# lenke182/flood-uav-video-segmentation

Measured on AMD Instinct MI355X. Metric: segmentation FPS @713x713 (PSPNet-ResNet50 keyframe + linear interp, frame_delta=5), higher is better.
Workload: dtype f32

## Files before the change

### flood_uav_video_segmentation_amd/csrc/kernels.h

```cpp
#pragma once
#include "common.h"

namespace fs {

struct ConvParams {
    const float* in;    int ld_in;
    const float* wgt;
    int ld_wgt;
    const float* scale;
    const float* shift;
    const float* res;   int ld_res;
    float* out;         int ld_out;
    int B, H, W, Cin;
    int Ho, Wo, Cout;
    int KH, KW, stride, pad, dil;
    const float* in2;   int ld_in2;
    int Cin2, stride2, H2, W2;
    int relu;
    int res_touch;
    int korder;
    int groups;
    long long g_in, g_wgt, g_out;
    const void* wgt3;
    unsigned plane_bytes;
    unsigned short* kv_k;
    unsigned short* kv_vt;
    int kv_N, kv_Npad, kv_heads;
    unsigned kv_plane_bytes;
    int kv_b;
};
int launch_conv_igemm(const ConvParams& p, hipStream_t s, int tile = 0);
const char* conv_igemm_tile_name(const ConvParams& p, int tile = 0);
int launch_split_bf16x3(const float* w, long long n, void* planes, hipStream_t s);

static inline int conv_out_size(int in, int k, int stride, int pad, int dil) { return (in + 2 * pad - dil * (k - 1) - 1) / stride + 1; }
static inline ConvParams conv2d_params(const float* in, int ld_in, const float* wgt, const float* scale, const float* shift, const float* res, int ld_res,
                                       float* out, int ld_out, int B, int H, int W, int Cin, int Cout, int KH, int KW, int stride, int pad, int dil,
                                       int relu, int korder) {
    ConvParams p{};
    p.in = in; p.ld_in = ld_in; p.wgt = wgt; p.scale = scale; p.shift = shift; p.res = res; p.ld_res = ld_res; p.out = out; p.ld_out = ld_out;
    p.B = B; p.H = H; p.W = W; p.Cin = Cin; p.Cout = Cout;
    p.Ho = conv_out_size(H, KH, stride, pad, dil);
    p.Wo = conv_out_size(W, KW, stride, pad, dil);
    p.KH = KH; p.KW = KW; p.stride = stride; p.pad = pad; p.dil = dil; p.relu = relu; p.korder = korder;
    return p;
}
static inline ConvParams gemm_params(const float* in, int ld_in, const float* w, float* out, int ld_out, int rows, int K, int N) {
    return conv2d_params(in, ld_in, w, nullptr, nullptr, nullptr, 0, out, ld_out, 1, rows, 1, K, N, 1, 1, 1, 0, 1, 0, 0);
}
static inline void attach_planes(ConvParams& p, const void* planes, size_t elems) {
    p.wgt3 = planes;
    p.plane_bytes = (unsigned)(elems * 2);
}

struct FrameSrc {
    const float* in;
    const float* in2;
    int B1;
    int ncrops, FH, FW;
    short cy[32], cx[32];
};
static inline FrameSrc frames_plain(const float* in, const float* in2, int B1) {
    FrameSrc f{};
    f.in = in;
    f.in2 = in2;
    f.B1 = B1;
    return f;
}

struct StemParams {
    FrameSrc src;
    const float* wgt;
    const float* scale; const float* shift;
    float* out; int ld_out;
    int B, H, W, Ho, Wo, Cout, KH, KW, stride, pad;
    int split;
};
int launch_stem_conv(const StemParams& p, hipStream_t s);
static inline StemParams stem_params(const FrameSrc& src, const float* wgt, const float* scale, const float* shift, float* out, int B, int H, int W,
                                     int Cout, int KH, int KW, int stride, int pad, int split) {
    StemParams p{};
    p.src = src; p.wgt = wgt; p.scale = scale; p.shift = shift; p.out = out; p.ld_out = Cout;
    p.B = B; p.H = H; p.W = W; p.Cout = Cout; p.KH = KH; p.KW = KW; p.stride = stride; p.pad = pad; p.split = split;
    p.Ho = conv_out_size(H, KH, stride, pad, 1);
    p.Wo = conv_out_size(W, KW, stride, pad, 1);
    return p;
}

int launch_maxpool3x3s2(const float* in, int ld_in, float* out, int ld_out, int B, int H, int W, int C,
                        int Ho, int Wo, hipStream_t s);

int launch_adaptive_avgpool(const float* in, int ld_in, float* out, int B, int H, int W, int C, int bin,
                            hipStream_t s);

int launch_ppm_pool_combine(const float* cell_mean, float* out1, float* out2, float* out3, int B, int C, hipStream_t s);

int launch_rowdot_1x1(const float* in, int ld_in, const float* wgt, const float* scale, const float* shift,
                      float* out, int ld_out, int M, int K, int N, int relu, hipStream_t s);
struct RowdotProblem { const float* in; const float* wgt; const float* scale; const float* shift; float* out; int M; };
struct RowdotBatch { RowdotProblem p[4]; };
int launch_rowdot_1x1_batch(const RowdotBatch& pb, int nprob, int ld_in, int ld_out, int K, int N, int relu, hipStream_t s);

int launch_upsample_into(const float* in, int hi, int wi, float* out, int ld_out, int B, int Ho, int Wo,
                         int C, int align_corners, hipStream_t s);

int launch_classifier_nchw(const float* in, int ld_in, const float* wgt , const float* bias,
                           float* out , int B, int HW, int C, int K, hipStream_t s);

int launch_pack_oihw_to_ohwi(const float* w, float* out, int O, int I, int KH, int KW, hipStream_t s);
int launch_pack_oihw_to_hwio(const float* w, float* out, int O, int I, int KH, int KW, hipStream_t s);
int launch_pack_oihw_chunk_major(const float* w, float* out, int O, int I, int KH, int KW, hipStream_t s);
int launch_pack_slice_tap_major(const float* w, float* out, int O, int I, int c0, int nc, int taps, hipStream_t s);
size_t ppm_term_scratch_floats(int B, int H, int C);
int launch_ppm_term_classify(const float* T, int ld, const float* const Z[4], const int bins[4], float* scratch, const float* scale,
                             const float* shift, int B, int H, int W, int C, int relu, const float* cls_w , const float* cls_b,
                             float* logits_nchw, int K, hipStream_t s);
int launch_concat_scaled_filters(const float* wa, const float* sa, const float* ha, int Ka, const float* wb, const float* sb, const float* hb,
                                 int Kb, float* out, float* shift_out, int O, hipStream_t s);
int launch_nchw_to_nhwc(const float* in, float* out, int ld_out, int B, int C, int HW, hipStream_t s);
int launch_nhwc_to_nchw(const float* in, int ld_in, float* out, int B, int C, int HW, hipStream_t s);

int launch_grid_sample_nchw(const float* in, int B, int C, int Hi, int Wi, const float* grid, int Hg, int Wg,
                            float* out, int align_corners, hipStream_t s);
int launch_grid_sample_nhwc(const float* in, int ld_in, int B, int C, int Hi, int Wi, const float* grid, int Hg,
                            int Wg, float* out, int ld_out, int align_corners, hipStream_t s);
int launch_resize_bilinear_nchw(const float* in, int BC, int Hi, int Wi, float* out, int Ho, int Wo,
                                int align_corners, hipStream_t s);
int launch_resize_bilinear_nhwc(const float* in, int ld_in, int B, int C, int Hi, int Wi, float* out, int ld_out,
                                int Ho, int Wo, int align_corners, hipStream_t s, int max_blocks = 16384);
int launch_blend(const float* a, float wa, const float* b, float wb, float* out, int64_t numel, hipStream_t s);

struct SegFuseArgs {
    const float* lo_prev;
    const float* lo_next;
    const float* const* grids_left;
    const float* const* grids_right;
    int K, h, w;
    int Hg, Wg;
    int H, W;
    int n;
    int no_warp;
    float* out_logits;
    uint8_t* out_mask;
    float* scratch;
    double* canvas;
    double* count;
    int cH, cW, y0, x0;
};
struct SegTailParams : SegFuseArgs {
    const float* weights;
};
int launch_seg_tail(const SegTailParams& p, hipStream_t s);

struct FeatTailParams {
    const float* f_prev;
    const float* f_next;
    const float* const* grids_left;
    const float* const* grids_right;
    const float* grid0;
    int C, fh, fw, Hg, Wg, H0, W0, n, no_warp;
    float* stack;
    float* scratch;
    const float* weights;
};
int launch_feat_tail(const FeatTailParams& p, hipStream_t s);

struct CropsFuseArgs {
    const float* lo_prev;
    const float* lo_next;
    const float* scratch;
    int nc;
    short cy[64], cx[64];
    int K, h, w, Hg, Wg, ch, cw, n, no_warp;
    double* canvas;
    uint8_t* mask;
    int H, W;
    float sy_lo, sx_lo, sy_g, sx_g;
};
struct CropsFuseParams : CropsFuseArgs {
    const float* weights;
};
int launch_crops_fuse(CropsFuseParams p, const float* grids, float* scratch, hipStream_t s);

int launch_ms_prepare(const float* raw, int H, int W, int new_h, int new_w, int PH, int PW, const float* mean, const float* std, float* out,
                      int flip, hipStream_t s);
struct MsFuseParams {
    const float* lo_plain;
    const float* lo_flip;
    int nc;
    short cy[64], cx[64];
    int K, h, w, ch, cw;
    int PH, PW, new_h, new_w;
    double* scaled;
    int pad_top, pad_left;
    float sy_lo, sx_lo;
};
int launch_ms_fuse(MsFuseParams p, double* pred, int H, int W, int scale_index, int nscales, uint8_t* mask, hipStream_t s);

int launch_argmax_u8(const float* in, int B, int K, int64_t HW, uint8_t* out, hipStream_t s);
int launch_resize_argmax_u8(const float* in, int B, int K, int Hi, int Wi, uint8_t* out, int Ho, int Wo,
                            hipStream_t s);
int launch_softmax_accumulate(const float* logits, int n, int K, int h, int w, double* canvas, double* count, int H, int W, int y0,
                              int x0, hipStream_t s);
int launch_canvas_finish(double* canvas, const double* count, int n, int K, int64_t HW, uint8_t* mask, hipStream_t s);
int launch_resize_crop(const float* in, int B, int K, int Hi, int Wi, int Hfull, int Wfull, int align_corners, float* logits,
                       uint8_t* mask, int Ho, int Wo, hipStream_t s);
int launch_canvas_resize_argmax(const double* canvas, int n, int K, int Hi, int Wi, uint8_t* mask, int Ho, int Wo, hipStream_t s);
struct CropGridParams {
    const float* grids[32];
    int ngrids, Hg, Wg;
    int H, W;
    int ncrops, fh, fw;
    int ng_total, g0;
    short bho[32], bwo[32], bh[32], bw[32];
    float off_h[32], off_w[32], den_h[32], den_w[32];
    float* out;
};
int launch_crop_grids(const CropGridParams& p, hipStream_t s);
int launch_colorize(const uint8_t* mask, const uint8_t* palette, int K, uint8_t* rgb, int64_t numel, hipStream_t s);
int launch_mv_to_grids(const int* mv, int n, int stride, int hb, int wb, int bs, int H, int W, int* owners, double* grid,
                       double* inv_grid, hipStream_t s);
int launch_block_match(const uint8_t* cur, const uint8_t* ref, int H, int W, int channels, int R, int lambda, int* mv, int* cost,
                       hipStream_t s);
int launch_block_match_modes(const uint8_t* cur, const uint8_t* ref, int H, int W, int channels, int R, int lambda, int intra_bias, int cut_permille,
                             int* mv, int* cost, int* activity, int* stats, hipStream_t s);
constexpr int WINDOW_MAX_FRAMES = 64;
int launch_window_weights(const int* const* stats, int n, float* weights, int* source, hipStream_t s);
int launch_frame_prepare(const uint8_t* frame, const uint8_t* u, const uint8_t* v, int format, int matrix, int full_range, int H, int W,
                         const float* mean, const float* std, float* out, int h, int w, hipStream_t s);
int launch_frame_compose(const uint8_t* mask, int h, int w, const uint8_t* palette, int K, const uint8_t* frame, const uint8_t* u, const uint8_t* v,
                         int format, int matrix, int full_range, int H, int W, uint8_t* out, uint8_t* out_u, uint8_t* out_v, int out_format,
                         int out_matrix, int out_full_range, hipStream_t s);
int launch_iou_hist(const uint8_t* pred, const uint8_t* target, int64_t numel, int K, int ignore_index,
                    long long* hist3K, hipStream_t s);
int launch_mask_confidence(const float* logits, int n, int K, int h, int w, uint8_t* mask, uint8_t* conf, int H, int W, hipStream_t s);
int launch_canvas_confidence(const double* canvas, int n, int K, int Hi, int Wi, uint8_t* mask, uint8_t* conf, int Ho, int Wo, hipStream_t s);
int launch_frame_report(const uint8_t* mask, const uint8_t* conf, int n, int H, int W, int K, int low, long long* out, hipStream_t s);

int region_rank_chunks(int H, int W);
int launch_mask_regions(const uint8_t* mask, int n, int H, int W, int K, int connectivity, int* labels, hipStream_t s);
int launch_region_table(const uint8_t* mask, const int* labels, const uint8_t* conf, int n, int H, int W, int K, int low, int max_regions,
                        long long* table, long long* counts, int* index, int* workspace, hipStream_t s);
int launch_region_filter(const uint8_t* mask, const int* index, const long long* table, int n, int H, int W, int K, int max_regions,
                         int min_area, uint8_t* out, int* votes, hipStream_t s);


int launch_patchify(const float* in, const float* in2, int B1, float* out, int B, int H, int W, int P, int gh, int gw, hipStream_t s);
int launch_vit_assemble(const float* emb, const float* cls, const float* pos, float* X, int B, int N, int D, hipStream_t s);
int launch_dec_assemble(const float* Y, const float* cls_emb, float* Z, int B, int N, int K, int D, hipStream_t s);
int launch_layernorm(const float* in, const float* gamma, const float* beta, float* out, int rows, int D, int rows_per_batch,
                     int drop_first, hipStream_t s);
size_t attention_scratch_floats(int B, int N, int heads);
int launch_attention_f32(const float* qkv, float* out, int B, int N, int heads, float scale, float* scratch, hipStream_t s);
size_t attention_split_floats(int B, int N, int heads);
int launch_attention_split(const float* qkv, float* out, int B, int N, int heads, float scale, float* scratch, float* planes, hipStream_t s, bool planes_ready = false);
int launch_splitk_combine(const float* part, int nsplit, const float* bias, const float* res, float* out, int rows, int N, hipStream_t s);
int launch_splitk_combine_ln(const float* part, int nsplit, const float* bias, const float* res, float* out, const float* gamma, const float* beta,
                             float* ln_out, int rows, int N, hipStream_t s);
int launch_mask_head(const float* pp, const float* cc, const float* gamma, const float* beta, float* out, int B, int N, int K,
                     int D, hipStream_t s);


int launch_winograd_filter(const float* w, float* U , int O, int I, int mt, hipStream_t s, int chunk_major = 0);
int launch_winograd_input(const float* in, int ld_in, float* V , int B, int H, int W, int C, int dil, int mt,
                          hipStream_t s);
int launch_winograd_output(const float* M , const float* scale, const float* shift, float* out, int ld_out, int B,
                           int H, int W, int N, int relu, int dil, int mt, hipStream_t s);
struct WinoLayout { bool tile_major; long long s_pos, s_tile; };
WinoLayout winograd_layout(int mt, long long T, int C);
static inline ConvParams winograd_gemm_params(const float* V, const float* U, float* M, int mt, int T, int Cin, int Cout) {
    ConvParams p = gemm_params(V, Cin, U, M, Cout, T, Cin, Cout);
    const WinoLayout a = winograd_layout(mt, T, Cin), o = winograd_layout(mt, T, Cout);
    p.ld_in = (int)a.s_tile;
    p.g_in = a.s_pos;
    p.ld_out = (int)o.s_tile;
    p.g_out = o.s_pos;
    p.groups = (mt + 2) * (mt + 2);
    p.g_wgt = (long long)Cout * Cin;
    return p;
}
static inline size_t wino_v_floats(int mt, size_t T, int Cin, size_t align) { return ((size_t)(mt + 2) * (mt + 2) * T * Cin + align - 1) / align * align; }
static inline size_t wino_vm_floats(int mt, size_t T, int Cin, int Cout, size_t align) {
    return wino_v_floats(mt, T, Cin, align) + (size_t)(mt + 2) * (mt + 2) * T * Cout;
}
static inline int winograd_tiles(int B, int H, int W, int dil, int mt) {
    return B * dil * dil * ((cdiv(H, dil) + mt - 1) / mt) * ((cdiv(W, dil) + mt - 1) / mt);
}
static inline double winograd_gemm_rows(int B, int H, int W, int dil, int mt) {
    return (double)(mt + 2) * (mt + 2) * (double)(cdiv(winograd_tiles(B, H, W, dil, mt), 64) * 64);
}
static inline int winograd_pick_m(int , int H, int W, int dil) {
    const int m = winograd_gemm_rows(1, H, W, dil, 6) < winograd_gemm_rows(1, H, W, dil, 4) ? 6 : 4;
    return winograd_gemm_rows(1, H, W, dil, 3) < winograd_gemm_rows(1, H, W, dil, m) ? 3 : m;
}
static inline int wino_m(int force, int H, int W, int dil) { return force ? force : winograd_pick_m(1, H, W, dil); }

size_t wino_fused_bank_floats(int Cin, int Cout);
bool wino_fused_supported(int Cin, int Cout, int KH, int KW, int stride, int pad, int dil);
int launch_wino4_filter_packed(const float* w, float* U, int O, int I, hipStream_t s, int chunk_major = 0);
int launch_wino4_fused(const float* in, int ld_in, const float* U, const float* scale, const float* shift, float* out, int ld_out, int B, int H,
                       int W, int Cin, int Cout, int relu, hipStream_t s, int variant = 0);

int launch_wino4_fused_pool(const float* in, int ld_in, const float* U, const float* scale, const float* shift, float* pool, int ld_pool, int B,
                            int H, int W, int Cin, int Cout, hipStream_t s);

}
```

### flood_uav_video_segmentation_amd/csrc/wino_fused.hip

```cpp
#include "kernels.h"
#include "winograd.h"

namespace fs {

__device__ __forceinline__ int wf_voff(int m, int k) {
    const int g = (0x78 >> ((m >> 1) & 6)) & 3;
    return m * 16 + 4 * ((k >> 2) ^ g) + (k & 3);
}

__device__ __forceinline__ void wf_bt(const float d[6], float t[6]) {
    const float s12 = d[1] + d[2], d12 = d[1] - d[2], s34 = d[3] + d[4], d43 = d[4] - d[3], d42 = d[4] - d[2], d31 = d[3] - d[1];
    t[0] = __builtin_fmaf(4.f, d[0], __builtin_fmaf(-5.f, d[2], d[4]));
    t[1] = __builtin_fmaf(-4.f, s12, s34);
    t[2] = __builtin_fmaf(4.f, d12, d43);
    t[3] = __builtin_fmaf(2.f, d31, d42);
    t[4] = __builtin_fmaf(-2.f, d31, d42);
    t[5] = __builtin_fmaf(4.f, d[1], __builtin_fmaf(-5.f, d[3], d[5]));
}
__device__ __forceinline__ void wf_at(const float m[6], float y[4]) {
    const float s12 = m[1] + m[2], d12 = m[1] - m[2], s34 = m[3] + m[4], d34 = m[3] - m[4];
    y[0] = (m[0] + s12) + s34;
    y[1] = __builtin_fmaf(2.f, d34, d12);
    y[2] = __builtin_fmaf(4.f, s34, s12);
    y[3] = __builtin_fmaf(8.f, d34, d12) + m[5];
}

__global__ __launch_bounds__(256) void wino4_filter_packed_kernel(const float* __restrict__ w, float* __restrict__ U, int O, int I, int chunk_major) {
    const int64_t total = (int64_t)O * I;
    const int ts = chunk_major ? 32 : 1;
    for (int64_t i = (int64_t)blockIdx.x * 256 + threadIdx.x; i < total; i += (int64_t)gridDim.x * 256) {
        const int o = (int)(i / I), c = (int)(i - (int64_t)o * I);
        const float* g = chunk_major ? w + (i >> 5) * 288 + (i & 31) : w + i * 9;
        double t[6][3];
#pragma unroll
        for (int s = 0; s < 3; ++s) {
            double col[6];
            Wino<4>::g(g[(0 * 3 + s) * ts], g[(1 * 3 + s) * ts], g[(2 * 3 + s) * ts], col);
#pragma unroll
            for (int r = 0; r < 6; ++r) t[r][s] = col[r];
        }
#pragma unroll
        for (int r = 0; r < 6; ++r) {
            double u[6];
            Wino<4>::g(t[r][0], t[r][1], t[r][2], u);
#pragma unroll
            for (int q = 0; q < 6; ++q) U[(((size_t)(r * 6 + q) * (I >> 4) + (c >> 4)) * O + o) * 16 + (c & 15)] = (float)u[q];
        }
    }
}

int launch_wino4_filter_packed(const float* w, float* U, int O, int I, hipStream_t s, int chunk_major) {
    FS_REQUIRE(I % 32 == 0 && O % 16 == 0, "wino_fused: Cin %% 32 == 0 and Cout %% 16 == 0 required (Cin=%d Cout=%d)", I, O);
    const int64_t total = (int64_t)O * I;
    hipLaunchKernelGGL(wino4_filter_packed_kernel, dim3((unsigned)std::min<int64_t>(cdiv64(total, 256), 65535)), dim3(256), 0, s, w, U, O, I, chunk_major);
    FS_HIP(hipGetLastError());
    return 0;
}

struct WinoFusedParams {
    const float* in;
    int ld_in;
    const float* U;
    const float* scale;
    const float* shift;
    float* out;
    int ld_out;
    int B, H, W, Cin, Cout, relu;
    int th, tw, T;
    float* pool;
    int ld_pool, Hp, Wp, nby, nbx;
};

#if defined(__HIP_DEVICE_COMPILE__)
__device__ __forceinline__ void wino4_epilogue(const f32x4 (&acc)[36], const WinoFusedParams& p, int tile, int n) {
    const float sc = p.scale ? p.scale[n] : 1.f, sh = p.shift ? p.shift[n] : 0.f;
    const __amdgpu_buffer_rsrc_t o_rsrc = __builtin_amdgcn_make_buffer_rsrc((void*)p.out, 0, (unsigned)((long long)p.B * p.H * p.W * p.ld_out * 4), 0x00020000);
    int tx = tile % p.tw, ty = (tile / p.tw) % p.th, b = tile / (p.tw * p.th);
#pragma unroll
    for (int r = 0; r < 4; ++r) {
        const bool tv = tile < p.T;
        const unsigned base = (unsigned)((((b * p.H + 4 * ty) * p.W + 4 * tx) * p.ld_out + n) * 4);
        float half[4][6];
#pragma unroll
        for (int x = 0; x < 6; ++x) {
            float col[6], y4[4];
#pragma unroll
            for (int y = 0; y < 6; ++y) col[y] = acc[y * 6 + x][r];
            wf_at(col, y4);
#pragma unroll
            for (int y = 0; y < 4; ++y) half[y][x] = y4[y];
        }
        const int ny = tv ? p.H - 4 * ty : 0, nx = p.W - 4 * tx;
#pragma unroll
        for (int y = 0; y < 4; ++y) {
            float o4[4];
            wf_at(half[y], o4);
#pragma unroll
            for (int x = 0; x < 4; ++x) {
                float v = __builtin_fmaf(o4[x], sc, sh);
                if (p.relu) v = fmaxf(v, 0.f);
                const unsigned vo = (y < ny && x < nx) ? base : 0x80000000u;
                __builtin_amdgcn_raw_buffer_store_b32(__builtin_bit_cast(unsigned, v), o_rsrc, vo, (unsigned)((y * p.W + x) * p.ld_out * 4), 0);
            }
        }
        ++tile;
        if (++tx == p.tw) {
            tx = 0;
            if (++ty == p.th) { ty = 0; ++b; }
        }
    }
}

__device__ __forceinline__ void wino4_epilogue_pool(const f32x4 (&acc)[36], const WinoFusedParams& p, int tb, int q, int n, int lane) {
    const float sc = p.scale ? p.scale[n] : 1.f, sh = p.shift ? p.shift[n] : 0.f;
    const int bx = tb % p.nbx, by = (tb / p.nbx) % p.nby, b = tb / (p.nbx * p.nby);
    const int R0 = 16 * by + 4 * q;
    float h[3][9];
    float carry[3] = {0.f, 0.f, 0.f};
#pragma unroll
    for (int r = 0; r < 4; ++r) {
        float half[4][6];
#pragma unroll
        for (int x = 0; x < 6; ++x) {
            float col[6], y4[4];
#pragma unroll
            for (int y = 0; y < 6; ++y) col[y] = acc[y * 6 + x][r];
            wf_at(col, y4);
#pragma unroll
            for (int y = 0; y < 4; ++y) half[y][x] = y4[y];
        }
        const int C0 = 16 * bx + 4 * r;
        float o[4][4];
#pragma unroll
        for (int y = 0; y < 4; ++y) {
            float o4[4];
            wf_at(half[y], o4);
#pragma unroll
            for (int x = 0; x < 4; ++x) {
                float v = __builtin_fmaf(o4[x], sc, sh);
                v = fmaxf(v, 0.f);
                o[y][x] = (R0 + y < p.H && C0 + x < p.W) ? v : 0.f;
            }
        }
        float rp[3][4];
#pragma unroll
        for (int x = 0; x < 4; ++x) {
            rp[0][x] = fmaxf(o[0][x], o[1][x]);
            rp[1][x] = fmaxf(fmaxf(o[1][x], o[2][x]), o[3][x]);
            rp[2][x] = o[3][x];
        }
#pragma unroll
        for (int sl = 0; sl < 3; ++sl) {
            h[sl][2 * r] = fmaxf(fmaxf(carry[sl], rp[sl][0]), rp[sl][1]);
            h[sl][2 * r + 1] = fmaxf(fmaxf(rp[sl][1], rp[sl][2]), rp[sl][3]);
            carry[sl] = rp[sl][3];
        }
    }
#pragma unroll
    for (int sl = 0; sl < 3; ++sl) h[sl][8] = carry[sl];
#pragma unroll
    for (int j = 0; j < 9; ++j) {
        const float below = __shfl_down(h[0][j], 16, 64);
        if (q < 3) h[2][j] = fmaxf(h[2][j], below);
    }
    int* pool = reinterpret_cast<int*>(p.pool);
#pragma unroll
    for (int sl = 0; sl < 3; ++sl) {
        if (sl == 0 && q != 0) continue;
        const int li = 2 * q + sl;
        const int pr = 8 * by + li;
        const bool row_rim = li == 0 || li == 8;
#pragma unroll
        for (int j = 0; j < 9; ++j) {
            const int pc = 8 * bx + j;
            if (pr >= p.Hp || pc >= p.Wp) continue;
            const int off = ((b * p.Hp + pr) * p.Wp + pc) * p.ld_pool + n;
            const int bits = __builtin_bit_cast(int, h[sl][j]);
            if (row_rim || j == 0 || j == 8) atomicMax(pool + off, bits);
            else pool[off] = bits;
        }
    }
}
#endif

template <int WM, int WN, bool POOL = false>
__global__ __launch_bounds__(64 * WM * WN, 2) void wino4_fused_kernel(WinoFusedParams p) {
#if defined(__HIP_DEVICE_COMPILE__)
    constexpr int NT = 16 * WM, NC = 16 * WN, NTHR = 64 * WM * WN;
    constexpr int ITEMS = NT * 16 / NTHR;
    static_assert(NT * 16 % NTHR == 0, "threads must divide the patches of a sub-chunk");
    constexpr int SUB = 36 * NT * 16;
    __shared__ __attribute__((aligned(1024))) float lds[2 * SUB];
    constexpr unsigned BAD = 0x40000000u;

    const int t = threadIdx.x, lane = t & 63, wv = __builtin_amdgcn_readfirstlane(t >> 6);
    const int wn = wv % WN, wm = wv / WN;
    const int ncb = p.Cout / NC;
    const int cb = blockIdx.x % ncb, tb = blockIdx.x / ncb;
    const int n0 = cb * NC;
    const int nstages = p.Cin >> 4;

    const __amdgpu_buffer_rsrc_t in_rsrc = __builtin_amdgcn_make_buffer_rsrc((void*)p.in, 0, (unsigned)((long long)p.B * p.H * p.W * p.ld_in * 4), 0x00020000);
    unsigned rowoff[ITEMS][6], coloff[ITEMS][6];
#pragma unroll
    for (int it = 0; it < ITEMS; ++it) {
        const int item = t + it * NTHR;
        int tx, ty, b;
        bool tv;
        if (POOL) {
            const int li = item >> 4;
            tx = 4 * (tb % p.nbx) + (li & 3);
            ty = 4 * ((tb / p.nbx) % p.nby) + (li >> 2);
            b = tb / (p.nbx * p.nby);
            tv = tx < p.tw && ty < p.th;
            if (!tv) tx = ty = 0;
        } else {
            const int tile = tb * NT + (item >> 4);
            tv = tile < p.T;
            const int tt = tv ? tile : 0;
            tx = tt % p.tw, ty = (tt / p.tw) % p.th, b = tt / (p.tw * p.th);
        }
        const int y0 = 4 * ty - 1, x0 = 4 * tx - 1;
#pragma unroll
        for (int k = 0; k < 6; ++k) {
            rowoff[it][k] = (tv && (unsigned)(y0 + k) < (unsigned)p.H) ? (unsigned)(((b * p.H + y0 + k) * p.W) * p.ld_in * 4) : BAD;
            coloff[it][k] = ((unsigned)(x0 + k) < (unsigned)p.W) ? (unsigned)(((x0 + k) * p.ld_in + (item & 15)) * 4) : BAD;
        }
    }

    const int m16 = lane & 15, q4 = lane >> 4;
    const __amdgpu_buffer_rsrc_t u_rsrc = __builtin_amdgcn_make_buffer_rsrc((void*)p.U, 0, (unsigned)((long long)36 * p.Cin * p.Cout * 4), 0x00020000);
    const unsigned b_voff = (unsigned)(((n0 + wn * 16 + m16) * 16 + 4 * q4) * 4);
    const unsigned u_chunk = (unsigned)p.Cout * 64u;
    const unsigned u_pos = (unsigned)(p.Cin >> 4) * u_chunk;
    const int a_off = wf_voff(wm * 16 + m16, 4 * q4);

    f32x4 acc[36];
#pragma unroll
    for (int g = 0; g < 36; ++g) acc[g] = f32x4(0.f);

    auto transform = [&](int stage, int buf) {
        {
#pragma unroll
            for (int it = 0; it < ITEMS; ++it) {
                const unsigned soff = (unsigned)(stage * 16 * 4);
                float d[6][6];
#pragma unroll
                for (int y = 0; y < 6; ++y)
#pragma unroll
                    for (int x = 0; x < 6; ++x)
                        d[y][x] = __builtin_bit_cast(float, __builtin_amdgcn_raw_buffer_load_b32(in_rsrc, rowoff[it][y] + coloff[it][x], soff, 0));
                float r[6][6];
#pragma unroll
                for (int x = 0; x < 6; ++x) {
                    float col[6], tc[6];
#pragma unroll
                    for (int y = 0; y < 6; ++y) col[y] = d[y][x];
                    wf_bt(col, tc);
#pragma unroll
                    for (int y = 0; y < 6; ++y) r[y][x] = tc[y];
                }
                float* dst = lds + buf * SUB + wf_voff((t + it * NTHR) >> 4, t & 15);
#pragma unroll
                for (int y = 0; y < 6; ++y) {
                    float o[6];
                    wf_bt(r[y], o);
#pragma unroll
                    for (int x = 0; x < 6; ++x) dst[(y * 6 + x) * (NT * 16)] = o[x];
                }
            }
        }
    };

    auto multiply = [&](int stage, int buf) {
        {
            const float* vsrc = lds + buf * SUB + a_off;
            const unsigned soff0 = (unsigned)stage * u_chunk;
#pragma unroll
            for (int g = 0; g < 36; g += 2) {
                const f32x4 a0 = *reinterpret_cast<const f32x4*>(vsrc + g * (NT * 16));
                const f32x4 a1 = *reinterpret_cast<const f32x4*>(vsrc + (g + 1) * (NT * 16));
                const f32x4 b0 = __builtin_bit_cast(f32x4, __builtin_amdgcn_raw_buffer_load_b128(u_rsrc, b_voff, soff0 + (unsigned)g * u_pos, 0));
                const f32x4 b1 = __builtin_bit_cast(f32x4, __builtin_amdgcn_raw_buffer_load_b128(u_rsrc, b_voff, soff0 + (unsigned)(g + 1) * u_pos, 0));
#pragma unroll
                for (int e = 0; e < 4; ++e) {
                    acc[g] = __builtin_amdgcn_mfma_f32_16x16x4f32(a0[e], b0[e], acc[g], 0, 0, 0);
                    acc[g + 1] = __builtin_amdgcn_mfma_f32_16x16x4f32(a1[e], b1[e], acc[g + 1], 0, 0, 0);
                }
            }
        }
    };

    transform(0, 0);
    for (int s = 0; s < nstages; ++s) {
        __syncthreads();
        const bool more = s + 1 < nstages;
        if (more) transform(s + 1, (s + 1) & 1);
        multiply(s, s & 1);
    }

    if constexpr (POOL) wino4_epilogue_pool(acc, p, tb, q4, n0 + wn * 16 + m16, lane);
    else wino4_epilogue(acc, p, tb * NT + wm * 16 + 4 * q4, n0 + wn * 16 + m16);
#endif
}

template <int PD>
__global__ __launch_bounds__(512, 2) void wino4_ws_kernel(WinoFusedParams p) {
#if defined(__HIP_DEVICE_COMPILE__)
    static_assert(18 % PD == 0, "PD must divide 18");
    constexpr int NT = 16, NC = 64, NB = 3;
    constexpr int SUB = 36 * NT * 16;
    __shared__ __attribute__((aligned(1024))) float lds[NB * SUB];
    constexpr unsigned BAD = 0x40000000u;

    const int t = threadIdx.x, lane = t & 63, wv = __builtin_amdgcn_readfirstlane(t >> 6);
    const int ncb = p.Cout / NC;
    const int nblk = ((p.T + NT - 1) / NT) * ncb, G = gridDim.x;
    const int n0 = ((int)blockIdx.x % ncb) * NC;
    const int nstages = p.Cin >> 4;
    const int total = ((nblk - (int)blockIdx.x + G - 1) / G) * nstages;

    if (wv >= 4) {
        const int tt = t - 256;
        const __amdgpu_buffer_rsrc_t in_rsrc = __builtin_amdgcn_make_buffer_rsrc((void*)p.in, 0, (unsigned)((long long)p.B * p.H * p.W * p.ld_in * 4), 0x00020000);
        unsigned voff[6][6];
        auto setup_block = [&](int blk) {
            const int tile = (blk / ncb) * NT + (tt >> 4);
            const bool tv = tile < p.T;
            const int tq = tv ? tile : 0;
            const int tx = tq % p.tw, ty = (tq / p.tw) % p.th, b = tq / (p.tw * p.th);
            const int y0 = 4 * ty - 1, x0 = 4 * tx - 1;
#pragma unroll
            for (int y = 0; y < 6; ++y) {
                const unsigned ro = (tv && (unsigned)(y0 + y) < (unsigned)p.H) ? (unsigned)(((b * p.H + y0 + y) * p.W) * p.ld_in * 4) : BAD;
#pragma unroll
                for (int x = 0; x < 6; ++x)
                    voff[y][x] = ro + (((unsigned)(x0 + x) < (unsigned)p.W) ? (unsigned)(((x0 + x) * p.ld_in + (tt & 15)) * 4) : BAD);
            }
        };
        float d[2][6][6];
        int ld_stage = 0, ld_blk = blockIdx.x;
        auto patch_load = [&](int set) {
            if (ld_stage == 0) setup_block(ld_blk);
            const unsigned soff = (unsigned)(ld_stage * 64);
#pragma unroll
            for (int y = 0; y < 6; ++y)
#pragma unroll
                for (int x = 0; x < 6; ++x) d[set][y][x] = __builtin_bit_cast(float, __builtin_amdgcn_raw_buffer_load_b32(in_rsrc, voff[y][x], soff, 0));
            if (++ld_stage == nstages) {
                ld_stage = 0;
                ld_blk += G;
            }
        };
        const int v_off = wf_voff(tt >> 4, tt & 15);
        auto transform = [&](int ring, int set) {
#pragma unroll
            for (int x = 0; x < 6; ++x) {
                float col[6], tc[6];
#pragma unroll
                for (int y = 0; y < 6; ++y) col[y] = d[set][y][x];
                wf_bt(col, tc);
#pragma unroll
                for (int y = 0; y < 6; ++y) d[set][y][x] = tc[y];
            }
            float* dst = lds + ring * SUB + v_off;
#pragma unroll
            for (int y = 0; y < 6; ++y) {
                float o[6];
                wf_bt(d[set][y], o);
#pragma unroll
                for (int x = 0; x < 6; ++x) dst[(y * 6 + x) * (NT * 16)] = o[x];
            }
        };
        int done = 0, ring = 0;
        auto produce = [&]() {
            if (done & 1) {
                if (done + 1 < total) patch_load(0);
                transform(ring, 1);
            } else {
                if (done + 1 < total) patch_load(1);
                transform(ring, 0);
            }
            ++done;
            if (++ring == NB) ring = 0;
        };
        patch_load(0);
        produce();
        for (int S = 0; S < total; ++S) {
            __syncthreads();
            while (done < total && done < S + NB) produce();
        }
        return;
    }

    const int wn = wv;
    const int m16 = lane & 15, q4 = lane >> 4;
    const __amdgpu_buffer_rsrc_t u_rsrc = __builtin_amdgcn_make_buffer_rsrc((void*)p.U, 0, (unsigned)((long long)36 * p.Cin * p.Cout * 4), 0x00020000);
    const unsigned b_voff = (unsigned)(((n0 + wn * 16 + m16) * 16 + 4 * q4) * 4);
    const unsigned u_chunk = (unsigned)p.Cout * 64u;
    const unsigned u_pos = (unsigned)(p.Cin >> 4) * u_chunk;
    const int a_off = wf_voff(m16, 4 * q4);

    f32x4 acc[36];
#pragma unroll
    for (int g = 0; g < 36; ++g) acc[g] = f32x4(0.f);
    f32x4 bq[PD][2];
    auto load_b = [&](int stage, int pair, int slot) {
        const unsigned so = (unsigned)stage * u_chunk + (unsigned)(2 * pair) * u_pos;
        bq[slot][0] = __builtin_bit_cast(f32x4, __builtin_amdgcn_raw_buffer_load_b128(u_rsrc, b_voff, so, 0));
        bq[slot][1] = __builtin_bit_cast(f32x4, __builtin_amdgcn_raw_buffer_load_b128(u_rsrc, b_voff, so + u_pos, 0));
    };
#pragma unroll
    for (int k = 0; k < PD; ++k) load_b(0, k, k);

    int blk = blockIdx.x, ms = 0, ring = 0;
    for (int S = 0; S < total; ++S) {
        __syncthreads();
        const float* vsrc = lds + ring * SUB + a_off;
        const bool more = S + 1 < total;
        const int ns = ms + 1 == nstages ? 0 : ms + 1;
        f32x4 aq[2][2];
        aq[0][0] = *reinterpret_cast<const f32x4*>(vsrc);
        aq[0][1] = *reinterpret_cast<const f32x4*>(vsrc + NT * 16);
#pragma unroll
        for (int k = 0; k < 18; ++k) {
            if (k + 1 < 18) {
                aq[(k + 1) & 1][0] = *reinterpret_cast<const f32x4*>(vsrc + (2 * k + 2) * (NT * 16));
                aq[(k + 1) & 1][1] = *reinterpret_cast<const f32x4*>(vsrc + (2 * k + 3) * (NT * 16));
            }
#pragma unroll
            for (int e = 0; e < 4; ++e) {
                acc[2 * k] = __builtin_amdgcn_mfma_f32_16x16x4f32(aq[k & 1][0][e], bq[k % PD][0][e], acc[2 * k], 0, 0, 0);
                __builtin_amdgcn_sched_barrier(0);
                acc[2 * k + 1] = __builtin_amdgcn_mfma_f32_16x16x4f32(aq[k & 1][1][e], bq[k % PD][1][e], acc[2 * k + 1], 0, 0, 0);
                __builtin_amdgcn_sched_barrier(0);
            }
            if (k + PD < 18) load_b(ms, k + PD, k % PD);
            else if (more) load_b(ns, k + PD - 18, k % PD);
            __builtin_amdgcn_sched_barrier(0);
        }
        if (++ring == NB) ring = 0;
        if (++ms == nstages) {
            wino4_epilogue(acc, p, (blk / ncb) * NT + 4 * q4, n0 + wn * 16 + m16);
#pragma unroll
            for (int g = 0; g < 36; ++g) acc[g] = f32x4(0.f);
            ms = 0;
            blk += G;
        }
    }
#endif
}

size_t wino_fused_bank_floats(int Cin, int Cout) { return (size_t)36 * Cin * Cout; }

bool wino_fused_supported(int Cin, int Cout, int KH, int KW, int stride, int pad, int dil) {
    return KH == 3 && KW == 3 && stride == 1 && pad == 1 && dil == 1 && Cin % 32 == 0 && Cin >= 32 && Cin <= 256 && Cout % 64 == 0;
}

int launch_wino4_fused(const float* in, int ld_in, const float* U, const float* scale, const float* shift, float* out, int ld_out, int B, int H,
                       int W, int Cin, int Cout, int relu, hipStream_t s, int variant) {
    FS_REQUIRE(wino_fused_supported(Cin, Cout, 3, 3, 1, 1, 1), "wino_fused: unsupported shape (Cin=%d Cout=%d)", Cin, Cout);
    FS_REQUIRE(variant == 0 || variant == 2 || variant == 3, "wino_fused: variant %d is not 0, 2 or 3", variant);
    FS_REQUIRE(ld_in >= Cin && ld_out >= Cout && ((uintptr_t)U & 15) == 0 && ((uintptr_t)in & 3) == 0, "wino_fused: bad strides / alignment");
    FS_REQUIRE((int64_t)B * H * W * ld_in * 4 < (int64_t)1 << 30 && (int64_t)B * H * W * ld_out * 4 < (int64_t)1 << 31,
               "wino_fused: input map must be smaller than 1 GiB, output smaller than 2 GiB");
    WinoFusedParams p{};
    p.in = in; p.ld_in = ld_in; p.U = U; p.scale = scale; p.shift = shift; p.out = out; p.ld_out = ld_out;
    p.B = B; p.H = H; p.W = W; p.Cin = Cin; p.Cout = Cout; p.relu = relu;
    p.th = cdiv(H, 4); p.tw = cdiv(W, 4);
    p.T = B * p.th * p.tw;
    const int ncb = Cout / 64;
    if (variant == 0) variant = (int64_t)cdiv(p.T, 16) * ncb > 512 ? 2 : 3;
    if (variant == 3) {
        const int nblk = cdiv(p.T, 16) * ncb;
        hipLaunchKernelGGL((wino4_ws_kernel<6>), dim3(std::min(nblk, 256 - 256 % ncb)), dim3(512), 0, s, p);
    }
    else hipLaunchKernelGGL((wino4_fused_kernel<1, 4>), dim3(cdiv(p.T, 16) * ncb), dim3(256), 0, s, p);
    FS_HIP(hipGetLastError());
    return 0;
}

int launch_wino4_fused_pool(const float* in, int ld_in, const float* U, const float* scale, const float* shift, float* pool, int ld_pool, int B,
                            int H, int W, int Cin, int Cout, hipStream_t s) {
    FS_REQUIRE(wino_fused_supported(Cin, Cout, 3, 3, 1, 1, 1), "wino_fused_pool: unsupported shape (Cin=%d Cout=%d)", Cin, Cout);
    FS_REQUIRE(ld_in >= Cin && ld_pool >= Cout && ((uintptr_t)U & 15) == 0 && ((uintptr_t)in & 3) == 0 && ((uintptr_t)pool & 3) == 0, "wino_fused_pool: bad strides / alignment");
    const int Hp = (H - 1) / 2 + 1, Wp = (W - 1) / 2 + 1;
    FS_REQUIRE((int64_t)B * H * W * ld_in * 4 < (int64_t)1 << 30 && (int64_t)B * Hp * Wp * ld_pool * 4 < (int64_t)1 << 31,
               "wino_fused_pool: input map must be smaller than 1 GiB, pooled map smaller than 2 GiB");
    WinoFusedParams p{};
    p.in = in; p.ld_in = ld_in; p.U = U; p.scale = scale; p.shift = shift; p.out = nullptr; p.ld_out = 0;
    p.B = B; p.H = H; p.W = W; p.Cin = Cin; p.Cout = Cout; p.relu = 1;
    p.th = cdiv(H, 4); p.tw = cdiv(W, 4);
    p.T = B * p.th * p.tw;
    p.pool = pool; p.ld_pool = ld_pool; p.Hp = Hp; p.Wp = Wp; p.nby = cdiv(p.th, 4); p.nbx = cdiv(p.tw, 4);
    FS_HIP(hipMemsetAsync(pool, 0, (size_t)B * Hp * Wp * ld_pool * sizeof(float), s));
    hipLaunchKernelGGL((wino4_fused_kernel<1, 4, true>), dim3((unsigned)(B * p.nby * p.nbx * (Cout / 64))), dim3(256), 0, s, p);
    FS_HIP(hipGetLastError());
    return 0;
}

}
```

Measured before the change: 1219.

## Add shared-transform Winograd kernel covering 128 output channels per block

Adds a 512-thread Winograd F(4,3) kernel in which one block transforms each 16-tile input stage once into double-buffered LDS and reuses it across 128 output channels, instead of 64. The input transform is split between two wave groups on alternating stages. A tail-balancing scheme launches leftover blocks as a half-position variant that splits the 36 Winograd positions across groups and reduces them through LDS, so the last wave fills more CUs. The kernel is used by default for large maps and for the pooled path when Cout is divisible by 128. This cuts redundant input transforms and loads, at the cost of one block per CU and an extra launch for the tail.

Result: no change. 1221 (median of 3 runs) (+0.1%).

```diff
diff --git a/flood_uav_video_segmentation_amd/csrc/kernels.h b/flood_uav_video_segmentation_amd/csrc/kernels.h
--- a/flood_uav_video_segmentation_amd/csrc/kernels.h
+++ b/flood_uav_video_segmentation_amd/csrc/kernels.h
@@ -296,6 +296,7 @@
 static inline int wino_m(int force, int H, int W, int dil) { return force ? force : winograd_pick_m(1, H, W, dil); }
 
 size_t wino_fused_bank_floats(int Cin, int Cout);
+bool wino_fused_shape_ok(int Cin, int Cout);
 bool wino_fused_supported(int Cin, int Cout, int KH, int KW, int stride, int pad, int dil);
 int launch_wino4_filter_packed(const float* w, float* U, int O, int I, hipStream_t s, int chunk_major = 0);
 int launch_wino4_fused(const float* in, int ld_in, const float* U, const float* scale, const float* shift, float* out, int ld_out, int B, int H,
diff --git a/flood_uav_video_segmentation_amd/csrc/wino_fused.hip b/flood_uav_video_segmentation_amd/csrc/wino_fused.hip
--- a/flood_uav_video_segmentation_amd/csrc/wino_fused.hip
+++ b/flood_uav_video_segmentation_amd/csrc/wino_fused.hip
@@ -50,7 +50,7 @@
 }
 
 int launch_wino4_filter_packed(const float* w, float* U, int O, int I, hipStream_t s, int chunk_major) {
-    FS_REQUIRE(I % 32 == 0 && O % 16 == 0, "wino_fused: Cin %% 32 == 0 and Cout %% 16 == 0 required (Cin=%d Cout=%d)", I, O);
+    FS_REQUIRE(I % (chunk_major ? 32 : 16) == 0 && O % 16 == 0, "wino_fused: Cin %% 16 == 0 (chunk-major: %% 32) and Cout %% 16 == 0 required (Cin=%d Cout=%d)", I, O);
     const int64_t total = (int64_t)O * I;
     hipLaunchKernelGGL(wino4_filter_packed_kernel, dim3((unsigned)std::min<int64_t>(cdiv64(total, 256), 65535)), dim3(256), 0, s, w, U, O, I, chunk_major);
     FS_HIP(hipGetLastError());
@@ -69,6 +69,7 @@
     int th, tw, T;
     float* pool;
     int ld_pool, Hp, Wp, nby, nbx;
+    int nwhole;
 };
 
 #if defined(__HIP_DEVICE_COMPILE__)
@@ -451,16 +452,157 @@
 #endif
 }
 
+template <bool POOL, bool HALF>
+__global__ __launch_bounds__(512, 1) void wino4_shared_kernel(WinoFusedParams p) {
+#if defined(__HIP_DEVICE_COMPILE__)
+    constexpr int NT = 16, NC = 128;
+    constexpr int SUB = 36 * NT * 16;
+    __shared__ __attribute__((aligned(1024))) float lds[2 * SUB];
+    constexpr unsigned BAD = 0x40000000u;
+
+    const int t = threadIdx.x, lane = t & 63, wv = __builtin_amdgcn_readfirstlane(t >> 6);
+    const int grp = wv >> 2, tt = t & 255;
+    const int ncb = p.Cout / NC;
+    constexpr int NP = HALF ? 18 : 36;
+    const int tb = HALF ? p.nwhole / ncb + (int)blockIdx.x / (2 * ncb) : (int)blockIdx.x / ncb;
+    const int n0 = HALF ? ((int)blockIdx.x % (2 * ncb)) * (NC / 2) : ((int)blockIdx.x % ncb) * NC;
+    const int cg = HALF ? wv & 3 : wv, pos0 = HALF ? 18 * (wv >> 2) : 0;
+    const int nstages = p.Cin >> 4;
+
+    const __amdgpu_buffer_rsrc_t in_rsrc = __builtin_amdgcn_make_buffer_rsrc((void*)p.in, 0, (unsigned)((long long)p.B * p.H * p.W * p.ld_in * 4), 0x00020000);
+    unsigned rowoff[6], coloff[6];
+    {
+        int tx, ty, b;
+        bool tv;
+        if (POOL) {
+            const int li = tt >> 4;
+            tx = 4 * (tb % p.nbx) + (li & 3);
+            ty = 4 * ((tb / p.nbx) % p.nby) + (li >> 2);
+            b = tb / (p.nbx * p.nby);
+            tv = tx < p.tw && ty < p.th;
+            if (!tv) tx = ty = 0;
+        } else {
+            const int tile = tb * NT + (tt >> 4);
+            tv = tile < p.T;
+            const int tq = tv ? tile : 0;
+            tx = tq % p.tw, ty = (tq / p.tw) % p.th, b = tq / (p.tw * p.th);
+        }
+        const int y0 = 4 * ty - 1, x0 = 4 * tx - 1;
+#pragma unroll
+        for (int k = 0; k < 6; ++k) {
+            rowoff[k] = (tv && (unsigned)(y0 + k) < (unsigned)p.H) ? (unsigned)(((b * p.H + y0 + k) * p.W) * p.ld_in * 4) : BAD;
+            coloff[k] = ((unsigned)(x0 + k) < (unsigned)p.W) ? (unsigned)(((x0 + k) * p.ld_in + (tt & 15)) * 4) : BAD;
+        }
+    }
+    const int v_off = wf_voff(tt >> 4, tt & 15);
+
+    const int m16 = lane & 15, q4 = lane >> 4;
+    const __amdgpu_buffer_rsrc_t u_rsrc = __builtin_amdgcn_make_buffer_rsrc((void*)p.U, 0, (unsigned)((long long)36 * p.Cin * p.Cout * 4), 0x00020000);
+    const unsigned b_voff = (unsigned)(((n0 + cg * 16 + m16) * 16 + 4 * q4) * 4);
+    const unsigned u_chunk = (unsigned)p.Cout * 64u;
+    const unsigned u_pos = (unsigned)(p.Cin >> 4) * u_chunk;
+    const int a_off = wf_voff(m16, 4 * q4);
+
+    f32x4 acc[36];
+#pragma unroll
+    for (int g = 0; g < 36; ++g) acc[g] = f32x4(0.f);
+
+    auto transform = [&](int stage, int buf) {
+        const unsigned soff = (unsigned)(stage * 16 * 4);
+        float d[6][6];
+#pragma unroll
+        for (int y = 0; y < 6; ++y)
+#pragma unroll
+            for (int x = 0; x < 6; ++x)
+                d[y][x] = __builtin_bit_cast(float, __builtin_amdgcn_raw_buffer_load_b32(in_rsrc, rowoff[y] + coloff[x], soff, 0));
+        float r[6][6];
+#pragma unroll
+        for (int x = 0; x < 6; ++x) {
+            float col[6], tc[6];
+#pragma unroll
+            for (int y = 0; y < 6; ++y) col[y] = d[y][x];
+            wf_bt(col, tc);
+#pragma unroll
+            for (int y = 0; y < 6; ++y) r[y][x] = tc[y];
+        }
+        float* dst = lds + buf * SUB + v_off;
+#pragma unroll
+        for (int y = 0; y < 6; ++y) {
+            float o[6];
+            wf_bt(r[y], o);
+#pragma unroll
+            for (int x = 0; x < 6; ++x) dst[(y * 6 + x) * (NT * 16)] = o[x];
+        }
+    };
+
+    auto multiply = [&](int stage, int buf) {
+        const float* vsrc = lds + buf * SUB + pos0 * (NT * 16) + a_off;
+        const unsigned soff0 = (unsigned)stage * u_chunk + (unsigned)pos0 * u_pos;
+#pragma unroll
+        for (int g = 0; g < NP; g += 2) {
+            const f32x4 a0 = *reinterpret_cast<const f32x4*>(vsrc + g * (NT * 16));
+            const f32x4 a1 = *reinterpret_cast<const f32x4*>(vsrc + (g + 1) * (NT * 16));
+            const f32x4 b0 = __builtin_bit_cast(f32x4, __builtin_amdgcn_raw_buffer_load_b128(u_rsrc, b_voff, soff0 + (unsigned)g * u_pos, 0));
+            const f32x4 b1 = __builtin_bit_cast(f32x4, __builtin_amdgcn_raw_buffer_load_b128(u_rsrc, b_voff, soff0 + (unsigned)(g + 1) * u_pos, 0));
+#pragma unroll
+            for (int e = 0; e < 4; ++e) {
+                acc[g] = __builtin_amdgcn_mfma_f32_16x16x4f32(a0[e], b0[e], acc[g], 0, 0, 0);
+                acc[g + 1] = __builtin_amdgcn_mfma_f32_16x16x4f32(a1[e], b1[e], acc[g + 1], 0, 0, 0);
+            }
+        }
+    };
+
+    if (grp < nstages) transform(grp, grp);
+    for (int s = 0; s < nstages; ++s) {
+        __syncthreads();
+        if (s >= 1 && s + 1 < nstages && ((s + 1) & 1) == grp) transform(s + 1, (s + 1) & 1);
+        multiply(s, s & 1);
+    }
+
+    if constexpr (HALF) {
+        f32x4* xch = reinterpret_cast<f32x4*>(lds) + cg * (18 * 64) + lane;
+        __syncthreads();
+        if (pos0) {
+#pragma unroll
+            for (int g = 0; g < 18; ++g) xch[g * 64] = acc[g];
+        }
+        __syncthreads();
+        if (pos0) return;
+#pragma unroll
+        for (int g = 0; g < 18; ++g) acc[18 + g] = xch[g * 64];
+    }
+
+    if constexpr (POOL) wino4_epilogue_pool(acc, p, tb, q4, n0 + cg * 16 + m16, lane);
+    else wino4_epilogue(acc, p, tb * NT + 4 * q4, n0 + cg * 16 + m16);
+#endif
+}
+
 size_t wino_fused_bank_floats(int Cin, int Cout) { return (size_t)36 * Cin * Cout; }
 
+bool wino_fused_shape_ok(int Cin, int Cout) { return Cin % 16 == 0 && Cin >= 16 && Cin <= 256 && Cout % 64 == 0; }
+
 bool wino_fused_supported(int Cin, int Cout, int KH, int KW, int stride, int pad, int dil) {
-    return KH == 3 && KW == 3 && stride == 1 && pad == 1 && dil == 1 && Cin % 32 == 0 && Cin >= 32 && Cin <= 256 && Cout % 64 == 0;
+    return KH == 3 && KW == 3 && stride == 1 && pad == 1 && dil == 1 && Cin % 32 == 0 && wino_fused_shape_ok(Cin, Cout);
+}
+
+static int wino_shared_whole(int blocks, int ncb) {
+    const int tail = cdiv((blocks * ncb) % 256, ncb);
+    return tail * ncb * 2 <= 256 ? (blocks - tail) * ncb : blocks * ncb;
+}
+
+template <bool POOL>
+static void launch_wino4_shared(WinoFusedParams& p, int blocks, int nwhole, hipStream_t s) {
+    p.nwhole = nwhole;
+    const int halves = 2 * (blocks * (p.Cout / 128) - nwhole);
+    if (nwhole) hipLaunchKernelGGL((wino4_shared_kernel<POOL, false>), dim3(nwhole), dim3(512), 0, s, p);
+    if (halves) hipLaunchKernelGGL((wino4_shared_kernel<POOL, true>), dim3(halves), dim3(512), 0, s, p);
 }
 
 int launch_wino4_fused(const float* in, int ld_in, const float* U, const float* scale, const float* shift, float* out, int ld_out, int B, int H,
                        int W, int Cin, int Cout, int relu, hipStream_t s, int variant) {
-    FS_REQUIRE(wino_fused_supported(Cin, Cout, 3, 3, 1, 1, 1), "wino_fused: unsupported shape (Cin=%d Cout=%d)", Cin, Cout);
-    FS_REQUIRE(variant == 0 || variant == 2 || variant == 3, "wino_fused: variant %d is not 0, 2 or 3", variant);
+    FS_REQUIRE(wino_fused_shape_ok(Cin, Cout), "wino_fused: unsupported shape (Cin=%d Cout=%d)", Cin, Cout);
+    FS_REQUIRE(variant == 0 || variant == 2 || variant == 3 || ((variant == 5 || variant == 6) && Cout % 128 == 0),
+               "wino_fused: variant %d is not 0, 2, 3 or (Cout %% 128 == 0 only) 5, 6", variant);
     FS_REQUIRE(ld_in >= Cin && ld_out >= Cout && ((uintptr_t)U & 15) == 0 && ((uintptr_t)in & 3) == 0, "wino_fused: bad strides / alignment");
     FS_REQUIRE((int64_t)B * H * W * ld_in * 4 < (int64_t)1 << 30 && (int64_t)B * H * W * ld_out * 4 < (int64_t)1 << 31,
                "wino_fused: input map must be smaller than 1 GiB, output smaller than 2 GiB");
@@ -470,8 +612,13 @@
     p.th = cdiv(H, 4); p.tw = cdiv(W, 4);
     p.T = B * p.th * p.tw;
     const int ncb = Cout / 64;
-    if (variant == 0) variant = (int64_t)cdiv(p.T, 16) * ncb > 512 ? 2 : 3;
-    if (variant == 3) {
+    const bool by_rule = variant == 0;
+    if (variant == 0) variant = (int64_t)cdiv(p.T, 16) * ncb > 512 ? (Cout % 128 == 0 ? 5 : 2) : 3;
+    if (variant == 5 || variant == 6) {
+        const int blocks = cdiv(p.T, 16);
+        launch_wino4_shared<false>(p, blocks, by_rule ? wino_shared_whole(blocks, Cout / 128) : variant == 5 ? blocks * (Cout / 128) : 0, s);
+    }
+    else if (variant == 3) {
         const int nblk = cdiv(p.T, 16) * ncb;
         hipLaunchKernelGGL((wino4_ws_kernel<6>), dim3(std::min(nblk, 256 - 256 % ncb)), dim3(512), 0, s, p);
     }
@@ -482,7 +629,7 @@
 
 int launch_wino4_fused_pool(const float* in, int ld_in, const float* U, const float* scale, const float* shift, float* pool, int ld_pool, int B,
                             int H, int W, int Cin, int Cout, hipStream_t s) {
-    FS_REQUIRE(wino_fused_supported(Cin, Cout, 3, 3, 1, 1, 1), "wino_fused_pool: unsupported shape (Cin=%d Cout=%d)", Cin, Cout);
+    FS_REQUIRE(wino_fused_shape_ok(Cin, Cout), "wino_fused_pool: unsupported shape (Cin=%d Cout=%d)", Cin, Cout);
     FS_REQUIRE(ld_in >= Cin && ld_pool >= Cout && ((uintptr_t)U & 15) == 0 && ((uintptr_t)in & 3) == 0 && ((uintptr_t)pool & 3) == 0, "wino_fused_pool: bad strides / alignment");
     const int Hp = (H - 1) / 2 + 1, Wp = (W - 1) / 2 + 1;
     FS_REQUIRE((int64_t)B * H * W * ld_in * 4 < (int64_t)1 << 30 && (int64_t)B * Hp * Wp * ld_pool * 4 < (int64_t)1 << 31,
@@ -494,7 +641,8 @@
     p.T = B * p.th * p.tw;
     p.pool = pool; p.ld_pool = ld_pool; p.Hp = Hp; p.Wp = Wp; p.nby = cdiv(p.th, 4); p.nbx = cdiv(p.tw, 4);
     FS_HIP(hipMemsetAsync(pool, 0, (size_t)B * Hp * Wp * ld_pool * sizeof(float), s));
-    hipLaunchKernelGGL((wino4_fused_kernel<1, 4, true>), dim3((unsigned)(B * p.nby * p.nbx * (Cout / 64))), dim3(256), 0, s, p);
+    if (Cout % 128 == 0) launch_wino4_shared<true>(p, B * p.nby * p.nbx, wino_shared_whole(B * p.nby * p.nbx, Cout / 128), s);
+    else hipLaunchKernelGGL((wino4_fused_kernel<1, 4, true>), dim3((unsigned)(B * p.nby * p.nbx * (Cout / 64))), dim3(256), 0, s, p);
     FS_HIP(hipGetLastError());
     return 0;
 }
```
